# PSilvestre/Clonos

Hardware: AMD Instinct MI355X
Metric: determinants/sec decode+delta-slice (higher is better)
Workload: dtype u8

## Files before the change

### clonos_amd/csrc/decode_fused.hip

```cpp
#include "dev_common.h"
#include "jser_device.h"
#include "jser_flat.h"
#include "handoff.h"

namespace clg {

constexpr uint32_t kZRowDw = kZRegion / 4;
constexpr uint32_t kZPitch = kZRowDw;
constexpr uint32_t kZRows = kZTile / kZRegion + 2;
constexpr uint32_t kZImgDw = kZRows * kZPitch;
constexpr uint32_t kZWin = 1024;
constexpr uint32_t kZEmitWin = 512;
constexpr int kZEmitPair = 1;
constexpr uint32_t kZCanon = 0xFFFFFFFFu;
constexpr uint32_t kZCanonLanes = 16;
constexpr int kZSer = -2;
constexpr uint32_t kZTiny = kZTinySpan;

template <int kCtrl>
__device__ __forceinline__ uint32_t dpp_mov(uint32_t v) {
  return (uint32_t)__builtin_amdgcn_mov_dpp((int)v, kCtrl, 0xF, 0xF, false);
}
__device__ __forceinline__ uint32_t wave_scan_u32(uint32_t v, uint32_t lane) {
  const uint32_t rl = lane & 15u;
// ... 398 lines not shown
template <bool J>
__device__ __forceinline__ Res merge_walk_r(const uint32_t* T, uint32_t re, uint32_t end_a, uint32_t e, const SpecR& s,
                                            const JL& jl) {
  return merge_walk_h(re, end_a, e, s, [&](uint32_t p, uint32_t* Lp, bool* w, uint32_t* why) -> bool {
    const uint32_t tg = zb8(T, p);
    uint32_t L = __builtin_amdgcn_ubfe(kZLutTrue, tg << 2, 4);
    *w = false;
    if (L == 15u || tg >= 8u) {
      int v;
      uint32_t y = 1u;
      if (tg >= 8u) {
        v = (int)kLenErr;
      } else if (tg == CLG_TAG_SERIALIZABLE) {
        if (J) {
          const uint32_t jv = jl_len(jl, p);
          v = jv ? (int)jv : (int)kLenErr;
        } else {
          v = (int)kLenErr;
          y = zbe32(T, p + 1) == 0xACED0005u ? 2u : 1u;
        }
      } else {
        v = tg == CLG_TAG_IGNORE_CHECKPOINT ? 13 : zlen_var(T, p, end_a, tg, 0);
      }
      if (v <= 0) {
        *why = y;
        return false;
      }
      L = (uint32_t)v;
      *w = true;
    }
    *Lp = L;
    return true;
  });
}

__device__ __forceinline__ Res merge_walk_lean(const uint32_t* T, uint32_t re, uint32_t end_a, uint32_t e,
                                               const SpecR& s) {
  Res r{{0, 0}, {0, 0}, e, 0, 0, 0};
  if (e >= re) return r;
  const uint32_t r0 = (re - 1u) & ~(kZRegion - 1u);
  uint32_t p = e, why = 0;
  Bits pb{0, 0}, pw{0, 0};
  auto run = [&](uint64_t sbw, uint64_t& pbw, uint64_t& pww, uint32_t lim) -> uint32_t {
    while (p < lim) {
      constexpr uint32_t kLo = 2u | 9u << 8 | 5u << 16;
      constexpr uint32_t kHi = 5u << 24;
      const uint32_t b = p & 63u;
      const uint64_t m = 1ull << b;
      const bool conv = (sbw & m) != 0ull && p >= s.bad;
      const uint32_t tg = zb8(T, p);
      const uint32_t L = __builtin_amdgcn_perm(kHi, kLo, min(tg, 12u)) & 0xFFu;
      if (conv || L == 0u || p + L > end_a) {
        if (conv) return 1u;
        int v;
        uint32_t y = 1u;
        if (tg >= 8u) {
          v = (int)kLenErr;
        } else if (tg == CLG_TAG_SERIALIZABLE) {
          v = (int)kLenErr;
          y = zbe32(T, p + 1) == 0xACED0005u ? 2u : 1u;
        } else if (L) {
          v = (int)kLenErr;
        } else {
          v = tg == CLG_TAG_IGNORE_CHECKPOINT ? 13 : zlen_var(T, p, end_a, tg, 0);
        }
        if (v <= 0 || p + (uint32_t)v > end_a || p + (uint32_t)v < p) {
          why = v <= 0 ? y : 1u;
          return 2u;
        }
        pbw |= m;
        pww |= m;
        p += (uint32_t)v;
        ++r.steps;
        continue;
      }
      pbw |= m;
      p += L;
      ++r.steps;
    }
    return 0u;
  };
  const uint32_t mid = re < r0 + 64u ? re : r0 + 64u;
  uint32_t st = run(s.sb.lo, pb.lo, pw.lo, mid);
  if (st == 0u) st = run(s.sb.hi, pb.hi, pw.hi, re);
  if (st == 1u) {
    const uint32_t i = p & 127u;
    r.bm = bor(pb, bge(s.sb, i));
    r.wb = bor(pw, bge(s.wb, i));
    r.exit = s.exit;
  } else if (st == 2u) {
    r.bad = why;
    r.exit = s.exit;
    r.bm = pb;
    r.wb = pw;
    r.fail = p;
  } else {
    r.bm = pb;
    r.wb = pw;
    r.exit = p;
  }
  return r;
}

__device__ __forceinline__ uint64_t ld_agent(const uint64_t* p) {
  return __hip_atomic_load(const_cast<uint64_t*>(p), __ATOMIC_RELAXED, __HIP_MEMORY_SCOPE_AGENT);
}
__device__ __forceinline__ uint32_t ld_agent32(const uint32_t* p) {
  return __hip_atomic_load(const_cast<uint32_t*>(p), __ATOMIC_RELAXED, __HIP_MEMORY_SCOPE_AGENT);
}
__device__ __forceinline__ void st_agent(uint64_t* p, uint64_t v) {
  __hip_atomic_store(p, v, __ATOMIC_RELAXED, __HIP_MEMORY_SCOPE_AGENT);
}
__device__ __forceinline__ void note_error(const FusedCtl& ctl, uint32_t span, uint64_t so) {
  if (ctl.span_err && so != ~0ull) atomicMin(reinterpret_cast<unsigned long long*>(ctl.span_err + span), (unsigned long long)so);
}
__device__ __forceinline__ void raise_abort(const FusedCtl& c, ZAbort reason, uint32_t t) {
  __hip_atomic_store(c.abort + kZAbortAny, 1u, __ATOMIC_RELAXED, __HIP_MEMORY_SCOPE_AGENT);
  __hip_atomic_fetch_max(c.abort + reason, ~t, __ATOMIC_RELAXED, __HIP_MEMORY_SCOPE_AGENT);
}

constexpr uint64_t kZSpinLimit = 1ull << 29;
__device__ __forceinline__ bool backoff(uint32_t& n, uint64_t t0) {
  for (uint32_t i = 0; i < n; ++i) __builtin_amdgcn_s_sleep(32);
  n = n < 16u ? n * 2u : 16u;
  return __builtin_amdgcn_s_memtime() - t0 < kZSpinLimit;
}

__device__ __forceinline__ uint64_t pack_cnt(uint32_t rec, uint32_t wide) { return (uint64_t)wide << 31 | rec; }

typedef uint32_t u32x4 __attribute__((ext_vector_type(4)));
constexpr int kZLoads = (int)(kZTile / 16 / 64);
struct StagePre {
  u32x4 v[kZLoads];
  u32x4 hv[2];
  uint32_t hb;
};
template <uint32_t kHaloMax = kZHalo>
struct StageGeom {
  uint32_t t1, halo, img_end;
  uint64_t after;
  bool near, far;
  __device__ __forceinline__ StageGeom(const TileDesc& td, const SpanDesc& sd, uint32_t t, uint32_t hi,
                                       const TileDesc* n1) {
    t1 = sd.first_tile + sd.n_tiles;
    after = td.span_off + td.len;
    const uint64_t rem = sd.len > after ? sd.len - after : 0;
    halo = rem < (uint64_t)kHaloMax ? (uint32_t)rem : kHaloMax;
    img_end = hi + halo;
    const bool next_ok = n1 && halo && t + 1 < t1 && n1->span_off == after && n1->len >= halo;
    near = kHaloMax <= 64u && next_ok;
    far = kHaloMax > 64u && next_ok;
  }
};
template <uint32_t kHaloMax = kZHalo>
__device__ __forceinline__ void stage_issue(const TileDesc& td, const SpanDesc& sd, const uint32_t t, const uint32_t lane,
                                            const uint32_t hi, const TileDesc* n1, StagePre& P) {
  static_assert(kHaloMax <= 64u * 16u * 2u - 32u, "halo words: two per lane");
  const StageGeom<kHaloMax> G(td, sd, t, hi, n1);
  const uint32_t words = (hi + 15) >> 4;
  const CLG_GLOBAL u32x4* src = gp(reinterpret_cast<const u32x4*>(td.abase));
#pragma unroll
  for (int i = 0; i < kZLoads; ++i) {
    const uint32_t w = lane + 64u * (uint32_t)i;
    P.v[i] = src[w < words ? w : words - 1u];
  }
  P.hb = 0;
  if (G.near && lane < G.halo) P.hb = gp(n1->abase)[n1->delta + lane];
  if (G.far) {
    const uint32_t nw = (n1->delta + G.halo + 15u) >> 4;
    const CLG_GLOBAL u32x4* src1 = gp(reinterpret_cast<const u32x4*>(n1->abase));
    P.hv[0] = lane < nw ? src1[lane] : u32x4{0, 0, 0, 0};
    P.hv[1] = lane + 64u < nw ? src1[lane + 64u] : u32x4{0, 0, 0, 0};
  }
}

template <uint32_t kHaloMax = kZHalo, uint32_t kRows = kZRows>
__device__ __forceinline__ void stage_finish(const TileDesc& td, const SpanDesc& sd, const uint32_t t,
                                             const TileDesc* __restrict__ tiles, uint32_t* s_img, const uint32_t lane,
                                             const uint32_t hi, const TileDesc* n1, const StagePre& P) {
  static_assert((kZTile + 15 + kHaloMax + 64 + 127) / 128 <= kRows, "image rows: tile + halo + zero pad");
  const StageGeom<kHaloMax> G(td, sd, t, hi, n1);
  const uint32_t t1 = G.t1, halo = G.halo, img_end = G.img_end;
  const uint64_t after = G.after;
  const bool near = G.near, far = G.far;
  const uint32_t hb = P.hb;
  const u32x4* hv = P.hv;
  {
    const uint32_t words = (hi + 15) >> 4;
#pragma unroll
    for (int i = 0; i < kZLoads; ++i) {
      const uint32_t w = lane + 64u * (uint32_t)i;
      if (w < words) {
        uint32_t* d = s_img + (w >> 3) * kZPitch + 4u * (w & 7u);
        d[0] = P.v[i].x;
        d[1] = P.v[i].y;
        d[2] = P.v[i].z;
        d[3] = P.v[i].w;
      }
    }
  }
  __syncthreads();
  {
    uint8_t* bb = reinterpret_cast<uint8_t*>(s_img);
    if (near) {
      if (lane < halo) bb[rb(hi + lane)] = (uint8_t)hb;
    } else if (far && ((hi - n1->delta) & 15u) == 0u) {
      const uint32_t nw = (n1->delta + halo + 15u) >> 4;
#pragma unroll
      for (uint32_t k = 0; k < 2; ++k) {
        const uint32_t c = lane + 64u * k;
        if (c >= nw) continue;
        const uint32_t at = hi - n1->delta + 16u * c;
        if (16u * c >= n1->delta) {
          uint32_t* d = s_img + rk(at >> 2);
          d[0] = hv[k].x;
          d[1] = hv[k].y;
          d[2] = hv[k].z;
          d[3] = hv[k].w;
        } else {
          const uint32_t w[4] = {hv[k].x, hv[k].y, hv[k].z, hv[k].w};
#pragma unroll
          for (uint32_t b = 0; b < 16; ++b)
            if (16u * c + b >= n1->delta) bb[rb(at + b)] = (uint8_t)(w[b >> 2] >> (8u * (b & 3u)));
        }
      }
    } else if (far) {
#pragma unroll
      for (uint32_t k = 0; k < 2; ++k) {
        const uint32_t c = lane + 64u * k;
        const uint32_t w[4] = {hv[k].x, hv[k].y, hv[k].z, hv[k].w};
#pragma unroll
        for (uint32_t b = 0; b < 16; ++b) {
          const uint32_t x = 16u * c + b;
          if (x >= n1->delta && x < n1->delta + halo) bb[rb(hi + x - n1->delta)] = (uint8_t)(w[b >> 2] >> (8u * (b & 3u)));
        }
      }
    } else {
      const TileDesc nn = halo ? tiles[t + 1] : td;
      if (kHaloMax > 64u && halo > 64u && nn.span_off == after && nn.len >= halo) {
        typedef uint32_t u32x4 __attribute__((ext_vector_type(4)));
        for (uint32_t c = lane; 16u * c < nn.delta + halo; c += 64) {
          const u32x4 v = gp(reinterpret_cast<const u32x4*>(nn.abase))[c];
          const uint32_t w[4] = {v.x, v.y, v.z, v.w};
#pragma unroll
          for (uint32_t b = 0; b < 16; ++b) {
            const uint32_t x = 16u * c + b;
            if (x >= nn.delta && x < nn.delta + halo) bb[rb(hi + x - nn.delta)] = (uint8_t)(w[b >> 2] >> (8u * (b & 3u)));
          }
        }
      } else {
        uint32_t k = t + 1;
        for (uint32_t i = lane; i < halo; i += 64) {
          const uint64_t o = after + i;
          while (k + 1 < t1 && o >= tiles[k].span_off + tiles[k].len) ++k;
          const TileDesc nt = tiles[k];
          bb[rb(hi + i)] = gp(nt.abase)[nt.delta + (uint32_t)(o - nt.span_off)];
        }
      }
    }
    bb[rb(img_end + lane)] = 0;
  }
  __syncthreads();
}


template <uint32_t kHaloMax = kZHalo, uint32_t kRows = kZRows>
__device__ __forceinline__ void stage_image(const TileDesc& td, const SpanDesc& sd, const uint32_t t,
                                            const TileDesc* __restrict__ tiles, uint32_t* s_img, const uint32_t lane,
                                            const uint32_t hi, const TileDesc* n1 = nullptr) {
  StagePre P;
  stage_issue<kHaloMax>(td, sd, t, lane, hi, n1, P);
  stage_finish<kHaloMax, kRows>(td, sd, t, tiles, s_img, lane, hi, n1, P);
}

struct ZTile {
  TileDesc td;
  SpanDesc sd;
  uint32_t lo, hi, end_a, rs, re;
  bool first, last;
};
__device__ __forceinline__ ZTile ztile_of(const TileDesc& td, const SpanDesc& sd, uint32_t t, uint32_t lane) {
  ZTile z;
  z.td = td;
  z.sd = sd;
  z.first = t == z.sd.first_tile;
  z.last = t + 1 == z.sd.first_tile + z.sd.n_tiles;
  z.lo = z.td.delta;
  z.hi = z.td.delta + z.td.len;
  const uint64_t ea = z.sd.len - z.td.span_off + z.td.delta;
  z.end_a = ea > 0xFFFFFF00ull ? 0xFFFFFF00u : (uint32_t)ea;
  const uint32_t r0 = lane * kZRegion;
  z.rs = r0 < z.lo ? z.lo : (r0 > z.hi ? z.hi : r0);
  z.re = r0 + kZRegion > z.hi ? z.hi : r0 + kZRegion;
  return z;
}
__device__ __forceinline__ ZTile ztile(const TileDesc* __restrict__ tiles, const SpanDesc* __restrict__ spans, uint32_t t,
                                       uint32_t lane) {
  const TileDesc td = tiles[t];
  return ztile_of(td, spans[td.span], t, lane);
}

constexpr uint32_t kZLmList = 2 * kZJBitsDw + kZJCap;
__device__ __forceinline__ void build_lm(const ZTile& z, uint32_t* T, uint32_t* list, const uint32_t lane) {
  const bool on = z.rs < z.re;
  const uint32_t r0 = lane * kZRegion;
  uint32_t c[kZRowDw];
  uint64_t cw0 = 0, cw1 = 0;
  constexpr bool kCols = true;
  const int32_t jmax = z.hi > z.lo ? ((int32_t)((z.hi - 1u) >> 7) - (int32_t)(lane >> 5)) >> 1 : -1;
  const uint32_t onm = jmax < 0 ? 0u : (jmax >= 31 ? 0xFFFFFFFFu : (2u << jmax) - 1u);
#pragma unroll
  for (uint32_t j = 0; j < kZRowDw; ++j) {
    const uint32_t x = kCols ? T[64u * j + lane] : T[lane * kZPitch + j];
    const uint32_t h = x & 0xF8F8F8F8u;
    const uint32_t zz = (h - 0x01010101u) & ~h & 0x80808080u;
    const uint32_t vm = __builtin_amdgcn_perm(zz << 8, zz, 0x090B080Au);
    c[j] = __builtin_amdgcn_perm(kLmHi, kLmLo, x) & vm;
    const uint64_t f = (uint64_t)((__builtin_amdgcn_perm(kLmCand, 0u, x) & vm) >> (7u - (j & 7u))) << (32u * ((j >> 3) & 1u));
    if (j < 16u) cw0 |= f; else cw1 |= f;
  }
  if (!kCols && !on) cw0 = cw1 = 0;
  const uint32_t nc = (uint32_t)(__popcll(cw0) + __popcll(cw1));
  const uint32_t incl = wave_scan_u32(nc, lane);
  const uint32_t n = min(lane63(incl), kZLmList);
  uint32_t idx = incl - nc;
#pragma unroll 1
  for (uint32_t hh = 0; hh < 2; ++hh) {
    uint64_t m = hh ? cw1 : cw0;
    while (m) {
      const uint32_t i = (uint32_t)__builtin_ctzll(m);
      m &= m - 1u;
      const uint32_t jj = 16u * hh + 8u * (i >> 5) + (i & 7u), b = (i >> 3) & 3u;
      const uint32_t a = kCols ? 4u * (64u * jj + lane) + b : r0 + 4u * jj + b;
      if (idx < kZLmList) list[idx] = (kCols ? a >= z.lo && a < z.hi : a >= z.rs && a < z.re) ? a : 0xFFFFu;
      ++idx;
    }
  }
  __syncthreads();
  for (uint32_t k = lane; k < n; k += 64) {
    const uint32_t a = list[k];
    const uint32_t code = a != 0xFFFFu ? lm_code(zlen_var(T, a, z.end_a, zb(T, a), 0u), true) : 0u;
    list[k] = a | code << 16;
  }
  __syncthreads();
#pragma unroll
  for (uint32_t j = 0; j < kZRowDw; ++j)
    if ((onm >> j) & 1u) T[64u * j + lane] = c[j];
  __syncthreads();
  for (uint32_t k = lane; k < n; k += 64) {
    const uint32_t e = list[k];
    if (e >> 16) lm8_set(T, e & 0xFFFFu, e >> 16);
  }
  if (on && z.end_a < r0 + kZRegion + 13u) {
    for (uint32_t a = z.end_a > r0 + 13u ? z.end_a - 13u : r0; a < r0 + kZRegion; ++a) {
      const uint32_t cc = lm8(T, a);
      if (a + (cc & 0x7Fu) > z.end_a) lm8_set(T, a, 0u);
    }
  }
}

struct GSpan {
  const TileDesc* tiles;
  uint32_t t, t1, lo;
  uint64_t so;
  __device__ uint32_t at(uint32_t a) const {
    const uint64_t o = so + (a - lo);
    uint32_t k = t;
    while (k + 1 < t1 && o >= tiles[k].span_off + tiles[k].len) ++k;
    const TileDesc d = tiles[k];
    return gp(d.abase)[d.delta + (uint32_t)(o - d.span_off)];
  }
};
struct GRec {
  GSpan g;
  uint32_t base;
  __device__ int operator()(uint64_t k) const { return (int)g.at(base + (uint32_t)k); }
};
__device__ __forceinline__ uint32_t fld_be32(const GRec& b, uint32_t k) {
  return (uint32_t)b(k) << 24 | (uint32_t)b(k + 1) << 16 | (uint32_t)b(k + 2) << 8 | (uint32_t)b(k + 3);
}
__device__ __forceinline__ int lm_true_slow(const GSpan& g, uint32_t p, uint32_t end_a, const JL& jl, uint32_t* wide) {
  const uint32_t tg = g.at(p);
  *wide = is_wide((int)tg);
  if (tg == CLG_TAG_SERIALIZABLE) {
    const uint32_t v = jl_len(jl, p);
    return v ? (int)v : -1;
  }
  const int64_t L = len_fields(GRec{g, p}, (int)tg, (uint64_t)(end_a - p));
  return (L > 0 && L <= 0x7FFFFFF0ll) ? (int)L : -1;
}

__device__ __forceinline__ Res merge_walk_lm(const uint32_t* M, uint32_t re, uint32_t end_a, uint32_t e, const SpecR& s,
                                             const JL& jl, const GSpan& g) {
  return merge_walk_h(re, end_a, e, s, [&](uint32_t p, uint32_t* Lp, bool* w, uint32_t* why) -> bool {
    const uint32_t cc = lm8(M, p);
    uint32_t L = cc & 0x7Fu, wu = cc >> 7;
    if (!L) {
      const int v = lm_true_slow(g, p, end_a, jl, &wu);
      if (v <= 0) {
        *why = 1;
        return false;
      }
      L = (uint32_t)v;
    }
    *Lp = L;
    *w = wu != 0;
    return true;
  });
}

template <bool J>
__device__ __forceinline__ uint32_t canon_walk_r(const uint32_t* T, uint32_t re, uint32_t end_a, uint32_t e,
                                                 const SpecR& s, const JL& jl, const GSpan& g) {
  if (e >= re) return e;
  const uint32_t r0 = (re - 1u) & ~(kZRegion - 1u);
  uint32_t p = e;
  while (p < re) {
    const uint32_t i = p - r0;
    if ((((i < 64u ? s.sb.lo : s.sb.hi) >> (i & 63u)) & 1ull) && p >= s.bad) return s.exit;
    uint32_t L;
    int v = 0;
    if (J && jl.lm) {
      const uint32_t c = lm8(jl.lm, p);
      L = c & 0x7Fu;
      if (c == 0x80u) {
        uint32_t w;
        v = lm_true_slow(g, p, end_a, jl, &w);
      }
    } else {
      bool w;
      L = spec_len_fast<J>(T, p, end_a, false, jl, &w);
      if (!L) {
        const uint32_t tg = zb8(T, p);
        if (tg == CLG_TAG_TIMER_TRIGGER || tg == CLG_TAG_SOURCE_CHECKPOINT) v = zlen_var(T, p, end_a, tg, 0u);
        else if (J && tg == CLG_TAG_SERIALIZABLE) v = (int)min(jl_len(jl, p), 0x7FFFFFFFu);
      }
    }
    if (!L) L = (v > 0 && v <= (int)kZTile) ? (uint32_t)v : 1u;
    p += L;
  }
  return p;
}

template <bool J>
__device__ __forceinline__ uint32_t canon_exit_r(const ZTile& z, const uint32_t* s_img, const SpecR& sp, uint32_t lane,
                                                 const JL& jl, const TileDesc* __restrict__ tiles, uint32_t t) {
  const GSpan g{tiles, t, z.sd.first_tile + z.sd.n_tiles, z.lo, z.td.span_off};
  const uint32_t last_l = z.hi > z.lo ? (z.hi - 1) >> 7 : 0;
  const uint32_t c0 = last_l >= kZCanonLanes - 1 ? last_l - (kZCanonLanes - 1) : 0;
  const bool on = lane >= c0 && z.rs < z.re;
  uint32_t cx = on ? sp.exit : z.rs, entry = kZCanon;
  for (int it = 0; it <= 64; ++it) {
    const uint32_t prev = wave_prev_u32(cx);
    const uint32_t want = lane <= c0 ? kZCanon : prev;
    const bool ch = want != entry;
    if (!__any(ch)) break;
    if (ch) {
      entry = want;
      cx = on ? canon_walk_r<J>(s_img, z.re, z.end_a, want, sp, jl, g) : want;
    }
  }
  return lane63(cx);
}

constexpr uint32_t kZWarmFlat = 1u << 31;
__device__ __forceinline__ uint32_t warm_start(uint32_t rs, uint32_t lo, uint32_t warm, uint32_t lane) {
  const uint32_t st = (lane >> 1) & 15u;
  const uint32_t w = (warm & kZWarmFlat) ? (warm & ~kZWarmFlat) : warm + 4u * st;
  return rs >= lo + w ? rs - w : lo;
}

template <bool J>
__device__ __forceinline__ ZAbort count_tile(const uint32_t t, const ZTile& z, const uint32_t e_true,
                                           const uint32_t must_exit, const FusedCtl& ctl, const uint32_t* s_img,
                                           const uint32_t lane, uint32_t* x_out, const JL& jl,
                                           const TileDesc* __restrict__ tiles = nullptr,
                                           const SpecR* walked = nullptr, uint64_t* cnt_out = nullptr,
                                           uint64_t* bm_out = nullptr, uint32_t* fail_out = nullptr) {
#define ZPHASE(i) \
  if (ctl.prof && lane == 0) ctl.prof[(uint64_t)t * 8 + (i)] = __builtin_amdgcn_s_memtime()
  ZPHASE(1);
  const uint32_t lo = z.lo, rs = z.rs, re = z.re, end_a = z.end_a;
  const uint32_t ws = warm_start(rs, lo, ctl.warm, lane), wsb = warm_start(lane * kZRegion + 64u, lo, ctl.warm, lane);
  const SpecR sp = walked ? *walked
                          : rs < re ? spec_walk_fast<J>(s_img, ws, wsb, rs, re, end_a, lane * kZRegion, jl, ctl.lean != 0u)
                                    : SpecR{{0, 0}, {0, 0}, rs, rs, 0};

  ZPHASE(2);
  const uint32_t guess = wave_prev_u32(sp.exit);
  uint32_t entry = lane == 0 ? e_true : guess;
  const GSpan g{tiles, t, z.sd.first_tile + z.sd.n_tiles, lo, z.td.span_off};
  auto merge = [&](uint32_t from) -> Res {
    if (rs >= re) return Res{{0, 0}, {0, 0}, from, 0, 0, 0};
    if (J && jl.lm) return merge_walk_lm(s_img, re, end_a, from, sp, jl, g);
    if (!J && ctl.lean) return merge_walk_lean(s_img, re, end_a, from, sp);
    return merge_walk_r<J>(s_img, re, end_a, from, sp, jl);
  };
  Res r = merge(entry);
  uint32_t steps0 = r.steps, steps_more = 0, iters = 0;
  uint32_t shift = 0;
  for (int it = 0; it <= 64; ++it) {
    const uint32_t prev = wave_prev_u32(r.exit);
    uint32_t want = lane == 0 ? e_true : prev;
    bool ch = want != entry;
    const uint64_t cm = __ballot(ch);
    if (!cm) break;
    ++iters;
    const uint32_t low = (uint32_t)__builtin_ctzll(cm);
    const uint32_t d = (uint32_t)__builtin_amdgcn_readlane((int)(want - entry), (int)low);
    if ((cm & (cm - 1)) == 0 && d == shift && lane > low) {
      want = entry + d;
      ch = true;
    }
    shift = (cm & (cm - 1)) == 0 ? d : 0u;
    if (ch) {
      entry = want;
      r = merge(want);
      steps_more += r.steps;
    }
  }
  if (ctl.prof) {
    uint32_t m0 = steps0, m1 = steps_more;
#pragma unroll
    for (int off = 32; off > 0; off >>= 1) {
      m0 = max(m0, (uint32_t)__shfl_xor(m0, off));
      m1 = max(m1, (uint32_t)__shfl_xor(m1, off));
    }
    if (lane == 0) ctl.prof[(uint64_t)t * 8 + 5] = (uint64_t)m0 | (uint64_t)m1 << 20 | (uint64_t)iters << 40;
  }
  const uint32_t x_true = lane63(r.exit);
  *x_out = x_true;
  const uint64_t badm = __ballot(r.bad != 0u);
  ZAbort reason = badm ? (__shfl(r.bad, (int)__builtin_ctzll(badm)) == 2u ? kZAbortSerializable : kZAbortBad) : kZAbortNone;
  if (z.last) {
    if (x_true != end_a) reason = reason ? reason : kZAbortEnd;
  } else if (must_exit != kZCanon && x_true != must_exit) {
    reason = reason ? reason : kZAbortExit;
  }
  if (reason && ctl.dbg) {
    uint32_t claim = 0;
    if (lane == 0) claim = atomicCAS(ctl.dbg + kZDbgClaim, 0u, 1u) == 0u ? 1u : 0u;
    if (__shfl(claim, 0)) {
      if (lane == 0) {
        ctl.dbg[kZDbgTile] = t; ctl.dbg[kZDbgReason] = reason; ctl.dbg[kZDbgMustExit] = must_exit;
        ctl.dbg[kZDbgXTrue] = x_true; ctl.dbg[kZDbgETrue] = e_true;
        ctl.dbg[kZDbgLo] = lo; ctl.dbg[kZDbgHi] = z.hi; ctl.dbg[kZDbgEndA] = end_a;
      }
      uint32_t* d = ctl.dbg + kZDbgLanes + kZDbgLaneWords * lane;
      d[0] = rs; d[1] = re; d[2] = sp.exit; d[3] = sp.bad; d[4] = sp.first; d[5] = 0; d[6] = entry;
      d[7] = r.exit | r.bad << 31;
    }
  }
  uint32_t fail_a = 0xFFFFFFFFu;
  if (reason == kZAbortBad && badm && ctl.span_err) {
    const uint32_t bl = (uint32_t)__builtin_ctzll(badm);
    fail_a = (uint32_t)__shfl((int)r.fail, (int)bl);
    if (lane > bl) {
      r.bm = Bits{0, 0};
      r.wb = Bits{0, 0};
    }
  }
  if (fail_out) *fail_out = fail_a;
  if (reason && reason != kZAbortExit && fail_a == 0xFFFFFFFFu) return reason;

  ZPHASE(3);
  const uint32_t pk = wave_sum_u32(bcount(r.bm) | bcount(r.wb) << 16);
  const uint32_t rec = pk & 0xFFFFu, wide = pk >> 16;
  if (lane == 0) gp(ctl.cnt)[t] = pack_cnt(rec, wide);
  if (cnt_out) *cnt_out = pack_cnt(rec, wide);
  if (bm_out) {
    bm_out[0] = r.bm.lo;
    bm_out[1] = r.bm.hi;
  }
  if (!bm_out) {
    typedef uint64_t u64x2 __attribute__((ext_vector_type(2)));
    u64x2 out_bits;
    out_bits.x = r.bm.lo;
    out_bits.y = r.bm.hi;
    gp(reinterpret_cast<u64x2*>(ctl.bits))[(uint64_t)t * 64 + lane] = out_bits;
  }
  ZPHASE(4);
#undef ZPHASE
  return reason;
}

__device__ __forceinline__ uint64_t wave_incl_scan(uint64_t v, uint32_t lane) {
#pragma unroll
  for (int off = 1; off < 64; off <<= 1) {
    const uint64_t y = __shfl_up(v, off);
    if ((int)lane >= off) v += y;
  }
  return v;
}

__global__ __launch_bounds__(256) void k_decode_scan1(FusedCtl ctl) {
  __shared__ uint64_t s_w[4];
  if (ld_agent32(ctl.abort + kZAbortAny)) return;
  const uint32_t tid = threadIdx.x, lane = tid & 63u, wv = tid >> 6;
  const uint32_t nt = ctl.n_tiles, blk = blockIdx.x, i0 = blk * kZScanBlock + tid * 4u;
  uint64_t v[4], sum = 0;
#pragma unroll
  for (int j = 0; j < 4; ++j) {
    v[j] = i0 + j < nt ? gp(ctl.cnt)[i0 + j] : 0ull;
    sum += v[j];
  }
  const uint64_t incl = wave_incl_scan(sum, lane);
  if (lane == 63u) s_w[wv] = incl;
  __syncthreads();
  uint64_t run = incl - sum;
  for (uint32_t k = 0; k < wv; ++k) run += s_w[k];
#pragma unroll
  for (int j = 0; j < 4; ++j) {
    if (i0 + j < nt) gp(ctl.base)[i0 + j] = run;
    run += v[j];
  }
  if (tid == 255u) gp(ctl.boff)[blk] = run;
}

__global__ __launch_bounds__(256) void k_decode_scan2(FusedCtl ctl, uint32_t n_blocks) {
  __shared__ uint64_t s_w[4];
  if (ld_agent32(ctl.abort + kZAbortAny)) return;
  const uint32_t tid = threadIdx.x, lane = tid & 63u, wv = tid >> 6, i0 = 4u * tid;
  uint64_t v[4], sum = 0;
#pragma unroll
  for (int j = 0; j < 4; ++j) {
    v[j] = i0 + j < n_blocks ? gp(ctl.boff)[i0 + j] : 0ull;
    sum += v[j];
  }
  const uint64_t incl = wave_incl_scan(sum, lane);
  if (lane == 63u) s_w[wv] = incl;
  __syncthreads();
  uint64_t run = incl - sum;
  for (uint32_t k = 0; k < wv; ++k) run += s_w[k];
#pragma unroll
  for (int j = 0; j < 4; ++j) {
    if (i0 + j < n_blocks) gp(ctl.boff)[i0 + j] = run;
    run += v[j];
// ... 361 lines not shown
        for (uint32_t j = 0; j < 9; ++j) d[j] = s_img[rk(k0 + j)];
#pragma unroll
        for (uint32_t j = 0; j < 8; ++j) x[j] = __builtin_amdgcn_alignbit(d[j + 1], d[j], sh);
        auto be32 = [&](uint32_t off) {
          return __builtin_bswap32(__builtin_amdgcn_alignbyte(x[(off >> 2) + 1], x[off >> 2], off & 3u));
        };
        const uint32_t tg = x[0] & 0xFFu;
        const bool ser = tg == CLG_TAG_SERIALIZABLE, tt = tg == CLG_TAG_TIMER_TRIGGER, sc = tg == CLG_TAG_SOURCE_CHECKPOINT;
        const uint32_t b13 = (x[3] >> 8) & 0xFFu, b21 = (x[5] >> 8) & 0xFFu, b22 = (x[5] >> 16) & 0xFFu;
        const bool tt_name = tt && b13 == 6u, sc_ref = sc && b22 != 0u;
        const uint32_t jlen = J && ser ? jl_len_bits(jl, a) : 0u;
        const uint32_t L = ser ? jlen : tt_name ? 18u + be32(14) : tt ? 14u : sc_ref ? 27u + be32(23) : sc ? 23u : 13u;
        const uint32_t var_off = ser ? 1u : tt_name ? 18u : sc_ref ? 27u : 0u;
        const int64_t v0 = ser ? (int64_t)L - 1 : (int64_t)((uint64_t)be32(5) << 32 | be32(9));
        if (fits || g < out.cap) o_v0[w0 + i] = v0;
        const uint64_t wi = wide + k;
        if (wi < out.wcap) {
          const uint32_t so = (uint32_t)(td.span_off + (a - lo));
          gp(out.w_idx)[wi] = (uint32_t)g;
          gp(out.w_rc)[wi] = ser ? 0 : (int32_t)be32(1);
          gp(out.w_v1)[wi] = sc ? (int64_t)((uint64_t)be32(13) << 32 | be32(17)) : 0;
          gp(out.w_var_off)[wi] = var_off ? so + var_off : 0u;
          gp(out.w_var_len)[wi] = var_off ? L - var_off : 0u;
          gp(out.w_sub)[wi] = (uint8_t)(tt ? b13 : sc ? (b21 | (sc_ref ? 0x80u : 0u)) : 0u);
        }
      }
    }
    wide += nwide;
    __syncthreads();
  }
}

template <bool J>
__global__ __launch_bounds__(64) void k_decode_emit(const TileDesc* __restrict__ tiles, const SpanDesc* __restrict__ spans,
                                                    FusedCtl ctl, DecodeOut out) {
  __shared__ EmitLds<J> L;
  const uint32_t t = blockIdx.x, lane = threadIdx.x;
  if (ld_agent32(ctl.abort + kZAbortAny)) return;
  if (ctl.lb_check && t && t % kZScanBlock == 0 && lane == 0) lookback_check(ctl, t / kZScanBlock);
  if (ctl.skip_bad && gp(ctl.span_bad)[tiles[t].span]) return;
  if (ctl.span_err && tiles[t].span_off > gp(ctl.span_err)[tiles[t].span]) return;
  emit_tile<J>(tiles, spans, ctl, out, t, lane, gp(ctl.base)[t] + gp(ctl.boff)[t / kZScanBlock], L);
}

constexpr uint64_t kZTinyDone = 1ull << 62;
__device__ __forceinline__ bool tiny_tile(const TileDesc& td, const SpanDesc& sd) {
  return sd.n_tiles == 1 && td.span_off == 0 && td.len > 0 && td.len <= kZTiny && td.len == sd.len;
}
__global__ __launch_bounds__(64) void k_decode_count_tiny(const TileDesc* __restrict__ tiles,
                                                          const SpanDesc* __restrict__ spans, FusedCtl ctl) {
  const uint32_t ti = blockIdx.x * 64 + threadIdx.x;
  if (ti >= ctl.n_tiles) return;
  const TileDesc td = tiles[ti];
  if (!tiny_tile(td, spans[td.span]) || (ctl.skip_bad && gp(ctl.span_bad)[td.span])) return;
  constexpr uint32_t kLeave = 3u;
  uint32_t why = 0, rec = 0, wide = 0;
  typedef uint32_t u32x4 __attribute__((ext_vector_type(4)));
  typedef uint64_t u64x2 __attribute__((ext_vector_type(2)));
  const CLG_GLOBAL u32x4* src = gp(reinterpret_cast<const u32x4*>(td.abase));
  auto* bits = gp(reinterpret_cast<u64x2*>(ctl.bits)) + (uint64_t)ti * 64;
  const uint32_t end = td.delta + td.len;
  uint32_t a = td.delta, wb = 0xFFFFFFFFu, cur = 0;
  u32x4 w{};
  uint64_t blo = 0, bhi = 0;
  constexpr uint32_t kLut = 2u | 9u << 4 | 5u << 8 | 13u << 24 | 5u << 28;
  while (a < end) {
    if ((a >> 4) != wb) {
      wb = a >> 4;
      w = src[wb];
    }
    const uint32_t q = a & 15u;
    const uint32_t dw = q < 8u ? (q < 4u ? w.x : w.y) : (q < 12u ? w.z : w.w);
    const uint32_t tg = (dw >> (8u * (q & 3u))) & 0xFFu;
    const uint32_t L = tg < 8u ? (kLut >> (4u * tg)) & 0xFu : 0u;
    if (!L) {
      why = (tg == CLG_TAG_SERIALIZABLE || tg == CLG_TAG_TIMER_TRIGGER || tg == CLG_TAG_SOURCE_CHECKPOINT) ? kLeave : kZAbortBad;
      break;
    }
    if (a + L > end) {
      why = kZAbortBad;
      break;
    }
    for (const uint32_t r = a >> 7; cur < r; ++cur) {
      u64x2 v;
      v.x = blo;
      v.y = bhi;
      bits[cur] = v;
      blo = bhi = 0;
    }
    const uint32_t i = a & 127u;
    if (i < 64u) blo |= 1ull << i; else bhi |= 1ull << (i - 64u);
    ++rec;
    wide += tg == CLG_TAG_IGNORE_CHECKPOINT ? 1u : 0u;
    a += L;
  }
  if (why == kLeave) return;
  if (why == 0u || ctl.span_err) {
    for (const uint32_t r = (end - 1) >> 7; cur <= r; ++cur) {
      u64x2 v;
      v.x = blo;
      v.y = bhi;
      bits[cur] = v;
      blo = bhi = 0;
    }
    gp(ctl.cnt)[ti] = pack_cnt(rec, wide);
  }
  if (why) {
    raise_abort(ctl, ZAbort(why), ti);
    if (ctl.span_bad) __hip_atomic_store(ctl.span_bad + td.span, 1u, __ATOMIC_RELAXED, __HIP_MEMORY_SCOPE_AGENT);
    note_error(ctl, td.span, (uint64_t)(a - td.delta));
  }
  gp(ctl.st_x)[ti] = kZTinyDone;
}

constexpr uint64_t kZExValid = 1ull << 63;
constexpr uint64_t kZExFail = 1ull << 62;

__device__ __forceinline__ void push_repair(const FusedCtl& ctl, uint32_t c) {
  gp(ctl.rep_flag)[c] = 1u;
  atomicAdd(ctl.rep + kZRepFiled, 1u);
}
__device__ __forceinline__ void mark_bad(const FusedCtl& ctl, ZAbort reason, uint32_t t, uint32_t span) {
  raise_abort(ctl, reason, t);
  if (ctl.span_bad) __hip_atomic_store(ctl.span_bad + span, 1u, __ATOMIC_RELAXED, __HIP_MEMORY_SCOPE_AGENT);
}
__device__ __forceinline__ uint32_t chunk_first(const FusedCtl& ctl, uint32_t c, uint32_t K, uint32_t G) {
  if (c >= G) return ctl.n_tiles;
  return ctl.chunk ? ctl.chunk[c] : min(ctl.n_tiles, c * K);
}
__device__ __forceinline__ void check_chunk(const FusedCtl& ctl, const TileDesc* __restrict__ tiles, uint32_t f,
                                            uint32_t ce, uint32_t lane) {
  const uint32_t span = tiles[f].span;
  uint32_t bad = 0xFFFFFFFFu;
  for (uint32_t i = f + lane; i < ce; i += 64) {
    if (tiles[i].span != span) break;
    if (!(ld_agent(&ctl.ex[i]) & kZExValid)) {
      bad = i;
      break;
    }
  }
  const uint64_t m = __ballot(bad != 0xFFFFFFFFu);
  if (m && lane == (uint32_t)__builtin_ctzll(m)) {
    mark_bad(ctl, kZAbortBad, bad, span);
    const uint64_t e = ld_agent(&ctl.ex[bad]);
    if (e & kZExFail) note_error(ctl, span, e & ~kZExFail);
  }
}

template <bool J>
__device__ __forceinline__ ZAbort count_staged(const TileDesc* __restrict__ tiles, const SpanDesc* __restrict__ spans,
                                                 const FusedCtl& ctl, uint32_t* s_img, uint32_t* s_j, uint32_t lane,
                                                 uint32_t t, const ZTile& z, uint64_t xs, uint32_t must_exit,
                                                 const SpecR* walked, uint64_t* x, uint64_t* cnt_out = nullptr,
                                                 uint64_t* bm_out = nullptr, uint64_t* fail_so = nullptr) {
  const uint32_t nt = ctl.n_tiles;
  const TileDesc n1 = tiles[t + 1 < nt ? t + 1 : t];
  const uint64_t ee = xs - z.td.span_off + z.lo;
  const uint32_t e_true = ee > 0xFFFFFF00ull ? 0xFFFFFF00u : (uint32_t)ee;
  JL jl{nullptr, nullptr, nullptr};
  JLPre pre{};
  if (J) pre = jl_prefetch(ctl, t, lane);
  stage_image(z.td, z.sd, t, tiles, s_img, lane, z.hi, &n1);
  if (J) build_lm(z, s_img, s_j, lane);
  if (J) jl = load_jl_map(ctl, t, s_j, lane, s_img, pre);
  uint32_t x_true, fa = 0xFFFFFFFFu;
  const ZAbort why = count_tile<J>(t, z, e_true, must_exit, ctl, s_img, lane, &x_true, jl, tiles, walked, cnt_out,
                                   bm_out, fail_so ? &fa : nullptr);
  *x = z.td.span_off + (x_true - z.lo);
  if (fail_so) *fail_so = fa != 0xFFFFFFFFu ? z.td.span_off + (fa - z.lo) : ~0ull;
  return why;
}

constexpr uint32_t kZWalkDisagree = 4;

__device__ __forceinline__ bool zero_tile_walk(const ZTile& z, uint64_t xs, const FusedCtl& ctl, uint32_t t,
                                               uint32_t lane, uint64_t* x) {
  const uint32_t words = (z.hi + 15) >> 4;
  const CLG_GLOBAL u32x4* src = gp(reinterpret_cast<const u32x4*>(z.td.abase));
  uint32_t any = 0;
#pragma unroll
  for (int i = 0; i < kZLoads; ++i) {
    const uint32_t w = lane + 64u * (uint32_t)i;
    const u32x4 v = src[w < words ? w : words - 1u];
    any |= v.x | v.y | v.z | v.w;
  }
  if (__any(any != 0u)) return false;
  const uint32_t e = (uint32_t)(xs - z.td.span_off) + z.lo;
  const uint32_t n = (z.hi - e + 1u) >> 1;
  const uint32_t r0 = lane * kZRegion;
  const uint64_t pat = (e & 1u) ? 0xAAAAAAAAAAAAAAAAull : 0x5555555555555555ull;
  auto word = [&](uint32_t b0) -> uint64_t {
    uint64_t m = pat;
    if (e > b0) m = e - b0 >= 64u ? 0ull : m & (~0ull << (e - b0));
    if (z.hi < b0 + 64u) m = z.hi <= b0 ? 0ull : m & ((1ull << (z.hi - b0)) - 1ull);
    return m;
  };
  typedef uint64_t u64x2 __attribute__((ext_vector_type(2)));
  u64x2 bits;
  bits.x = word(r0);
  bits.y = word(r0 + 64u);
  gp(reinterpret_cast<u64x2*>(ctl.bits))[(uint64_t)t * 64 + lane] = bits;
  if (lane == 0) gp(ctl.cnt)[t] = pack_cnt(n, 0);
  *x = z.td.span_off + (e + 2u * n - z.lo);
  return true;
}

__device__ __forceinline__ bool wrong_entry(const FusedCtl& ctl, uint32_t c, uint32_t f) {
  const uint64_t e = ld_agent(&ctl.ent[c]);
  if (!pk_state(e) || f == 0) return false;
  const uint64_t xe = ld_agent(&ctl.ex[f - 1]);
  return !(xe & kZExValid) || (xe & ~kZExValid) != pk_val(e);
}

template <bool J>
__device__ __forceinline__ bool serve_chunk(const TileDesc* __restrict__ tiles, const SpanDesc* __restrict__ spans,
                                            const FusedCtl& ctl, uint32_t* s_img, uint32_t* s_j, uint32_t lane,
                                            uint32_t c, uint32_t f, uint32_t ce, uint32_t* walk_end) {
  if (f == 0 || f >= ce || tiles[f].span_off == 0) return true;
  if (f >= *walk_end) {
    const uint64_t xe = ld_agent(&ctl.ex[f - 1]);
    if (!(xe & kZExValid)) {
      if (lane == 0) mark_bad(ctl, kZAbortBad, f - 1, tiles[f].span);
      return true;
    }
    uint64_t xs = xe & ~kZExValid;
    const uint64_t e = ld_agent(&ctl.ent[c]);
    const uint64_t taken = pk_state(e) ? pk_val(e) : pk_val(ld_agent(&ctl.st_x[f - 1]));
    if (xs != taken) {
      uint32_t disagree = 0;
      for (uint32_t t = f; t < ctl.n_tiles; ++t) {
        const ZTile z = ztile(tiles, spans, t, lane);
        *walk_end = t + 1;
        uint64_t x = xs, fso = ~0ull;
        ZAbort why = kZAbortNone;
        bool zero = false;
        if (!z.last && xs >= z.td.span_off + z.td.len) {
          typedef uint64_t u64x2 __attribute__((ext_vector_type(2)));
          gp(reinterpret_cast<u64x2*>(ctl.bits))[(uint64_t)t * 64 + lane] = u64x2{0, 0};
          if (lane == 0) gp(ctl.cnt)[t] = 0;
        } else if (!z.last && zero_tile_walk(z, xs, ctl, t, lane, &x)) {
          zero = true;
        } else {
          why = count_staged<J>(tiles, spans, ctl, s_img, s_j, lane, t, z, xs, kZCanon, nullptr, &x, nullptr, nullptr,
                                &fso);
          __syncthreads();
          if (why == kZAbortBad && lane == 0) note_error(ctl, z.td.span, fso);
        }
        if (why) {
          if (lane == 0) {
            mark_bad(ctl, why, t, z.td.span);
            st_agent(&ctl.ex[t], why == kZAbortBad && fso != ~0ull ? kZExFail | fso : 0ull);
          }
          break;
        }
        const uint64_t xv = kZExValid | x;
        uint32_t old = 0;
        if (lane == 0) {
          const uint64_t o = ld_agent(&ctl.ex[t]);
          old = o == xv ? 1u : (o & kZExValid) ? 2u : 0u;
          st_agent(&ctl.ex[t], xv);
          if (ctl.dbg) {
            uint64_t* w = reinterpret_cast<uint64_t*>(ctl.dbg + kZDbgTiles) + 2 * (uint64_t)t;
            w[0] = xs;
            w[1] = 2ull << 60 | (uint64_t)blockIdx.x << 32 | (uint64_t)(f & 0xFFFFFF) << 4 | old;
          }
        }
        old = __shfl(old, 0);
        if (old == 1u || z.last) break;
        if (old == 2u && !zero && ++disagree > kZWalkDisagree) {
          if (lane == 0) {
            mark_bad(ctl, kZAbortExit, t, z.td.span);
            if (ctl.dbg) {
              ctl.dbg[kZDbgWalkMark] = kZDbgWalkGaveUp; ctl.dbg[kZDbgWalkFrom] = f; ctl.dbg[kZDbgWalkAt] = t;
              ctl.dbg[kZDbgWalkEntry] = (uint32_t)(xs - z.td.span_off);
              ctl.dbg[kZDbgWalkExit] = (uint32_t)(x - z.td.span_off); ctl.dbg[kZDbgWalkSpan] = z.td.span;
              ctl.dbg[kZDbgWalkDisagree] = disagree;
            }
          }
          return false;
        }
        xs = x;
      }
    }
  }
  check_chunk(ctl, tiles, f, ce, lane);
  return true;
}

template <bool J>
constexpr int kZCountWaves = J ? 3 : 4;
template <bool J>
__global__ __launch_bounds__(64) __attribute__((amdgpu_waves_per_eu(kZCountWaves<J>))) void k_decode_count(const TileDesc* __restrict__ tiles, const SpanDesc* __restrict__ spans,
                                                     FusedCtl ctl) {
  __shared__ uint32_t s_img[kZImgDw];
  __shared__ uint32_t s_j[J ? 2 * kZJBitsDw + kZJCap : 1];
  const uint32_t lane = threadIdx.x, nt = ctl.n_tiles;
  JL jl{nullptr, nullptr, nullptr};
  const uint32_t K = (nt + gridDim.x - 1) / gridDim.x;
  const uint32_t t0 = chunk_first(ctl, blockIdx.x, K, gridDim.x), t1 = chunk_first(ctl, blockIdx.x + 1, K, gridDim.x);
  uint32_t x_pub = kZCanon;
  SpecR sp_last{{0, 0}, {0, 0}, 0, 0, 0};
  if (t0 < t1) {
    const ZTile z = ztile(tiles, spans, t1 - 1, lane);
    if (!z.last && t1 < nt) {
      stage_image(z.td, z.sd, t1 - 1, tiles, s_img, lane, z.hi);
      if (J) build_lm(z, s_img, s_j, lane);
      if (J) jl = load_jl_map(ctl, t1 - 1, s_j, lane, s_img, jl_prefetch(ctl, t1 - 1, lane));
      const uint32_t ws = warm_start(z.rs, z.lo, ctl.warm, lane);
      const uint32_t wsb = warm_start(lane * kZRegion + 64u, z.lo, ctl.warm, lane);
      sp_last = z.rs < z.re ? spec_walk_fast<J>(s_img, ws, wsb, z.rs, z.re, z.end_a, lane * kZRegion, jl, ctl.lean != 0u)
                            : SpecR{{0, 0}, {0, 0}, z.rs, z.rs, 0};
      x_pub = canon_exit_r<J>(z, s_img, sp_last, lane, jl, tiles, t1 - 1);
      if (x_pub < z.hi) {
        if (lane == 0) atomicAdd(ctl.rep + kZRepCanonEarly, 1u);
        x_pub = z.hi;
      }
      if (lane == 0) st_agent(&ctl.st_x[t1 - 1], pk_word(2u, (uint64_t)z.td.span_off + (x_pub - z.lo)));
      __syncthreads();
    }
  }
  uint64_t x_prev = 0;
  uint32_t bad_span = 0xFFFFFFFFu;
  uint32_t sus_span = 0xFFFFFFFFu;
  for (uint32_t t = t0; t < t1; ++t) {
    const ZTile z = ztile(tiles, spans, t, lane);
    if (z.td.span == bad_span) continue;
    if (!J && ctl.tiny && z.first && z.last && z.td.len <= kZTiny && gp(ctl.st_x)[t] == kZTinyDone)
      continue;
    if (ctl.prof && lane == 0) ctl.prof[(uint64_t)t * 8] = __builtin_amdgcn_s_memtime();
    uint64_t xs;
    if (z.first) {
      xs = z.td.span_off;
    } else if (t > t0) {
      xs = x_prev;
    } else {
      uint64_t v;
      uint32_t nb = 1;
      const uint64_t w0 = __builtin_amdgcn_s_memtime();
      for (;;) {
        v = ld_agent(&ctl.st_x[t - 1]);
        if (pk_state(v) && pk_val(v) >= z.td.span_off) break;
        if (pk_state(v) && ctl.dbg && lane == 0) {
          if (atomicAdd(ctl.dbg + kZDbgSkipN, 1u) == 0u) {
            ctl.dbg[kZDbgSkipTile] = t; ctl.dbg[kZDbgSkipWordLo] = (uint32_t)v; ctl.dbg[kZDbgSkipWordHi] = (uint32_t)(v >> 32);
            ctl.dbg[kZDbgSkipOff] = (uint32_t)z.td.span_off; ctl.dbg[kZDbgSkipPolls] = nb;
          }
        }
        if (ld_agent32(ctl.abort + kZAbortTimeout)) return;
        if (!backoff(nb, w0)) {
          if (lane == 0) raise_abort(ctl, kZAbortTimeout, t);
          return;
        }
      }
      xs = pk_val(v) + (ctl.perturb & 0xFFFFu);
      sus_span = z.td.span;
      if (lane == 0) st_agent(&ctl.ent[blockIdx.x], pk_word(2u, xs));
    }
    const bool reuse = t + 1 == t1 && x_pub != kZCanon;
    uint64_t x;
    uint64_t fso = ~0ull;
    const ZAbort why = count_staged<J>(tiles, spans, ctl, s_img, s_j, lane, t, z, xs, t + 1 == t1 ? x_pub : kZCanon,
                                       reuse ? &sp_last : nullptr, &x, nullptr, nullptr, &fso);
    if (why == kZAbortNone || why == kZAbortExit) {
      x_prev = x;
      if (lane == 0) {
        st_agent(&ctl.ex[t], kZExValid | x);
        if (ctl.dbg) {
          uint64_t* w = reinterpret_cast<uint64_t*>(ctl.dbg + kZDbgTiles) + 2 * (uint64_t)t;
          w[0] = xs;
          w[1] = 1ull << 60 | (uint64_t)blockIdx.x << 32 | (uint64_t)(t0 & 0xFFFFFF) << 4 | why;
        }
        if (why == kZAbortExit) {
          uint32_t c = blockIdx.x + 1;
          while (chunk_first(ctl, c + 1, K, gridDim.x) == t1) ++c;
          push_repair(ctl, c);
        }
      }
    } else {
      const bool soft = why != kZAbortSerializable && z.td.span == sus_span;
      if (lane == 0) {
        if (soft) {
          push_repair(ctl, blockIdx.x);
          if (why == kZAbortBad && fso != ~0ull) st_agent(&ctl.ex[t], kZExFail | fso);
        } else {
          mark_bad(ctl, why, t, z.td.span);
          if (why == kZAbortBad) note_error(ctl, z.td.span, fso);
        }
      }
      if (!soft && !ctl.span_bad) return;
      if (soft)
        x_prev = z.td.span_off + z.td.len;
      else
        bad_span = z.td.span;
    }
    __syncthreads();
  }
}

template <bool J>
__global__ __launch_bounds__(64) void k_decode_repair(const TileDesc* __restrict__ tiles, const SpanDesc* __restrict__ spans,
                                                      FusedCtl ctl) {
  __shared__ uint32_t s_img[kZImgDw];
  __shared__ uint32_t s_j[J ? 2 * kZJBitsDw + kZJCap : 1];
  if (ld_agent32(ctl.abort + kZAbortTimeout) || ld_agent32(ctl.abort + kZAbortSerializable) ||
      ld_agent32(ctl.abort + kZAbortOverflow))
    return;
  const uint32_t G = gridDim.x, b = blockIdx.x, lane = threadIdx.x, K = (ctl.n_tiles + G - 1) / G;
  const uint32_t fb = chunk_first(ctl, b, K, G);
  if (fb >= chunk_first(ctl, b + 1, K, G)) return;
  auto need = [&](uint32_t c, uint32_t f) -> bool { return gp(ctl.rep_flag)[c] || wrong_entry(ctl, c, f); };
  if (!need(b, fb)) return;
  const uint32_t span = tiles[fb].span;
  for (uint32_t hi = b; hi > 0;) {
    const uint32_t lo = hi > 64u ? hi - 64u : 0u, k = lo + lane;
    const bool in = k < hi;
    const uint32_t ft = in ? chunk_first(ctl, k, K, G) : 0u;
    const uint32_t kt = in ? chunk_first(ctl, k + 1, K, G) : 0u;
    const bool empty = in && kt == ft, same = in && !empty && tiles[ft].span == span;
    if (__any(same && need(k, ft))) return;
    if (!__all(!in || empty || same)) break;
    hi = lo;
  }
  uint32_t walk_end = 0;
  for (uint32_t c = b; c < G; ++c) {
    const uint32_t f = chunk_first(ctl, c, K, G), ce = chunk_first(ctl, c + 1, K, G);
    if (f >= ce) continue;
    if (tiles[f].span != span) break;
    if (!gp(ctl.rep_flag)[c]) {
      if (!wrong_entry(ctl, c, f)) continue;
      if (lane == 0 && (ld_agent(&ctl.ex[f - 1]) & kZExValid)) atomicAdd(ctl.rep + kZRepServed, 1u);
    }
    if (!serve_chunk<J>(tiles, spans, ctl, s_img, s_j, lane, c, f, ce, &walk_end)) break;
  }
}

constexpr uint32_t kZAggSet = 2u, kZAggBad = 3u;

__device__ __forceinline__ void decode_small_tiles(const TileDesc* __restrict__ tiles,
                                                   const SpanDesc* __restrict__ spans, uint32_t nt, const FusedCtl& ctl,
                                                   const DecodeOut& out, uint64_t* agg, uint64_t* agg_next,
                                                   uint64_t* res) {
  __shared__ EmitLds<false, true> L;
  const uint32_t t = blockIdx.x, lane = threadIdx.x;
  for (uint32_t j = t + nt * lane; j < kZSmallAggWords; j += 64u * nt) agg_next[j] = 0;
  const ZTile z = ztile(tiles, spans, t, lane);
  const TileDesc n1 = tiles[t + 1 < nt ? t + 1 : t];
  stage_image(z.td, z.sd, t, tiles, L.img, lane, z.hi, &n1);
  const JL jl{nullptr, nullptr, nullptr};
  const uint32_t ws = warm_start(z.rs, z.lo, ctl.warm, lane), wsb = warm_start(lane * kZRegion + 64u, z.lo, ctl.warm, lane);
  const SpecR sp = z.rs < z.re ? spec_walk_fast<false>(L.img, ws, wsb, z.rs, z.re, z.end_a, lane * kZRegion, jl,
                                                       ctl.lean != 0u)
                               : SpecR{{0, 0}, {0, 0}, z.rs, z.rs, 0};
  uint64_t xs = z.td.span_off;
  bool bad = false;
  if (!z.first) {
    uint64_t v = 0;
    if (lane == 0) {
      const uint64_t w0 = __builtin_amdgcn_s_memtime();
      while (!pk_state(v = ld_agent(&agg[nt + t - 1]))) {
        __builtin_amdgcn_s_sleep(1);
        if (__builtin_amdgcn_s_memtime() - w0 >= kZSpinLimit) {
          v = pk_word(kZAggBad, 0);
          break;
        }
      }
    }
    v = ((uint64_t)__builtin_amdgcn_readfirstlane((uint32_t)(v >> 32)) << 32) |
        (uint32_t)__builtin_amdgcn_readfirstlane((uint32_t)v);
    bad = pk_state(v) == kZAggBad;
    xs = pk_val(v) + (ctl.perturb & 0xFFFFu);
  }
  uint64_t c = 0, x = 0, bm[2] = {0, 0};
  if (!bad) {
    const uint64_t ee = xs - z.td.span_off + z.lo;
    const uint32_t e_true = ee > 0xFFFFFF00ull ? 0xFFFFFF00u : (uint32_t)ee;
    uint32_t x_true;
    const ZAbort why = count_tile<false>(t, z, e_true, kZCanon, ctl, L.img, lane, &x_true, jl, tiles, &sp, &c, bm);
    x = z.td.span_off + (x_true - z.lo);
    bad = why != kZAbortNone;
  }
  if (lane == 0) {
    st_agent(&agg[nt + t], pk_word(bad ? kZAggBad : kZAggSet, x));
    st_agent(&agg[t], pk_word(bad ? kZAggBad : kZAggSet, c));
  }
  uint64_t pre = 0;
  bool any_bad = bad;
  for (uint32_t j0 = 0; j0 < t && !any_bad; j0 += 64) {
    const uint32_t j = j0 + lane;
    uint64_t v = 0;
    if (j < t) {
      const uint64_t w0 = __builtin_amdgcn_s_memtime();
      while (!pk_state(v = ld_agent(&agg[j]))) {
        __builtin_amdgcn_s_sleep(1);
        if (__builtin_amdgcn_s_memtime() - w0 >= kZSpinLimit) {
          v = pk_word(kZAggBad, 0);
          break;
        }
      }
    }
    any_bad = __any(pk_state(v) == kZAggBad);
    uint64_t cj = pk_val(v);
#pragma unroll
    for (int off = 32; off > 0; off >>= 1) cj += __shfl_xor(cj, off);
    pre += cj;
  }
  if (any_bad) {
    if (lane == 0) __hip_atomic_store(res + kZSmallFailed, 1ull, __ATOMIC_RELAXED, __HIP_MEMORY_SCOPE_SYSTEM);
    return;
  }
  emit_tile<false, true>(tiles, spans, ctl, out, t, lane, pre, L, bm);
  if (lane == 0) {
    uint64_t* ck = res + small_check_at(ctl.n_spans, t);
    ck[kZCheckEntryExit] = (uint64_t)(uint32_t)xs | (uint64_t)(uint32_t)x << 32;
    ck[kZCheckBase] = pre;
    ck[kZCheckCount] = c;
// ... 539 lines not shown
```

Baseline: 98.38 billion.

## Stage only the canonical tail of the last tile and raise count-kernel occupancy

Result: no change. 99.55 billion, median of 5 (+1.2%).

```diff
diff --git a/clonos_amd/csrc/decode_fused.hip b/clonos_amd/csrc/decode_fused.hip
--- a/clonos_amd/csrc/decode_fused.hip
+++ b/clonos_amd/csrc/decode_fused.hip
@@ -574,16 +574,17 @@
     far = kHaloMax > 64u && next_ok;
   }
 };
-template <uint32_t kHaloMax = kZHalo>
+template <uint32_t kHaloMax = kZHalo, int kLoads = kZLoads>
 __device__ __forceinline__ void stage_issue(const TileDesc& td, const SpanDesc& sd, const uint32_t t, const uint32_t lane,
-                                            const uint32_t hi, const TileDesc* n1, StagePre& P) {
+                                            const uint32_t hi, const TileDesc* n1, StagePre& P, const uint32_t w0 = 0) {
+  static_assert(kLoads <= kZLoads, "the words a lane holds");
   static_assert(kHaloMax <= 64u * 16u * 2u - 32u, "halo words: two per lane");
   const StageGeom<kHaloMax> G(td, sd, t, hi, n1);
   const uint32_t words = (hi + 15) >> 4;
   const CLG_GLOBAL u32x4* src = gp(reinterpret_cast<const u32x4*>(td.abase));
 #pragma unroll
-  for (int i = 0; i < kZLoads; ++i) {
-    const uint32_t w = lane + 64u * (uint32_t)i;
+  for (int i = 0; i < kLoads; ++i) {
+    const uint32_t w = w0 + lane + 64u * (uint32_t)i;
     P.v[i] = src[w < words ? w : words - 1u];
   }
   P.hb = 0;
@@ -596,10 +597,11 @@
   }
 }
 
-template <uint32_t kHaloMax = kZHalo, uint32_t kRows = kZRows>
+template <uint32_t kHaloMax = kZHalo, uint32_t kRows = kZRows, int kLoads = kZLoads>
 __device__ __forceinline__ void stage_finish(const TileDesc& td, const SpanDesc& sd, const uint32_t t,
                                              const TileDesc* __restrict__ tiles, uint32_t* s_img, const uint32_t lane,
-                                             const uint32_t hi, const TileDesc* n1, const StagePre& P) {
+                                             const uint32_t hi, const TileDesc* n1, const StagePre& P,
+                                             const uint32_t w0 = 0) {
   static_assert((kZTile + 15 + kHaloMax + 64 + 127) / 128 <= kRows, "image rows: tile + halo + zero pad");
   const StageGeom<kHaloMax> G(td, sd, t, hi, n1);
   const uint32_t t1 = G.t1, halo = G.halo, img_end = G.img_end;
@@ -610,8 +612,8 @@
   {
     const uint32_t words = (hi + 15) >> 4;
 #pragma unroll
-    for (int i = 0; i < kZLoads; ++i) {
-      const uint32_t w = lane + 64u * (uint32_t)i;
+    for (int i = 0; i < kLoads; ++i) {
+      const uint32_t w = w0 + lane + 64u * (uint32_t)i;
       if (w < words) {
         uint32_t* d = s_img + (w >> 3) * kZPitch + 4u * (w & 7u);
         d[0] = P.v[i].x;
@@ -686,13 +688,13 @@
 }
 
 
-template <uint32_t kHaloMax = kZHalo, uint32_t kRows = kZRows>
+template <uint32_t kHaloMax = kZHalo, uint32_t kRows = kZRows, int kLoads = kZLoads>
 __device__ __forceinline__ void stage_image(const TileDesc& td, const SpanDesc& sd, const uint32_t t,
                                             const TileDesc* __restrict__ tiles, uint32_t* s_img, const uint32_t lane,
-                                            const uint32_t hi, const TileDesc* n1 = nullptr) {
+                                            const uint32_t hi, const TileDesc* n1 = nullptr, const uint32_t w0 = 0) {
   StagePre P;
-  stage_issue<kHaloMax>(td, sd, t, lane, hi, n1, P);
-  stage_finish<kHaloMax, kRows>(td, sd, t, tiles, s_img, lane, hi, n1, P);
+  stage_issue<kHaloMax, kLoads>(td, sd, t, lane, hi, n1, P, w0);
+  stage_finish<kHaloMax, kRows, kLoads>(td, sd, t, tiles, s_img, lane, hi, n1, P, w0);
 }
 
 struct ZTile {
@@ -864,12 +866,16 @@
   return p;
 }
 
+__device__ __forceinline__ uint32_t canon_first_lane(const ZTile& z) {
+  const uint32_t last_l = z.hi > z.lo ? (z.hi - 1) >> 7 : 0;
+  return last_l >= kZCanonLanes - 1 ? last_l - (kZCanonLanes - 1) : 0;
+}
+
 template <bool J>
 __device__ __forceinline__ uint32_t canon_exit_r(const ZTile& z, const uint32_t* s_img, const SpecR& sp, uint32_t lane,
                                                  const JL& jl, const TileDesc* __restrict__ tiles, uint32_t t) {
   const GSpan g{tiles, t, z.sd.first_tile + z.sd.n_tiles, z.lo, z.td.span_off};
-  const uint32_t last_l = z.hi > z.lo ? (z.hi - 1) >> 7 : 0;
-  const uint32_t c0 = last_l >= kZCanonLanes - 1 ? last_l - (kZCanonLanes - 1) : 0;
+  const uint32_t c0 = canon_first_lane(z);
   const bool on = lane >= c0 && z.rs < z.re;
   uint32_t cx = on ? sp.exit : z.rs, entry = kZCanon;
   for (int it = 0; it <= 64; ++it) {
@@ -898,13 +904,14 @@
                                            const uint32_t lane, uint32_t* x_out, const JL& jl,
                                            const TileDesc* __restrict__ tiles = nullptr,
                                            const SpecR* walked = nullptr, uint64_t* cnt_out = nullptr,
-                                           uint64_t* bm_out = nullptr, uint32_t* fail_out = nullptr) {
+                                           uint64_t* bm_out = nullptr, uint32_t* fail_out = nullptr,
+                                           const uint32_t walked_from = 0) {
 #define ZPHASE(i) \
   if (ctl.prof && lane == 0) ctl.prof[(uint64_t)t * 8 + (i)] = __builtin_amdgcn_s_memtime()
   ZPHASE(1);
   const uint32_t lo = z.lo, rs = z.rs, re = z.re, end_a = z.end_a;
   const uint32_t ws = warm_start(rs, lo, ctl.warm, lane), wsb = warm_start(lane * kZRegion + 64u, lo, ctl.warm, lane);
-  const SpecR sp = walked ? *walked
+  const SpecR sp = walked && lane >= walked_from ? *walked
                           : rs < re ? spec_walk_fast<J>(s_img, ws, wsb, rs, re, end_a, lane * kZRegion, jl, ctl.lean != 0u)
                                     : SpecR{{0, 0}, {0, 0}, rs, rs, 0};
 
@@ -1572,7 +1579,8 @@
                                                  const FusedCtl& ctl, uint32_t* s_img, uint32_t* s_j, uint32_t lane,
                                                  uint32_t t, const ZTile& z, uint64_t xs, uint32_t must_exit,
                                                  const SpecR* walked, uint64_t* x, uint64_t* cnt_out = nullptr,
-                                                 uint64_t* bm_out = nullptr, uint64_t* fail_so = nullptr) {
+                                                 uint64_t* bm_out = nullptr, uint64_t* fail_so = nullptr,
+                                                 const uint32_t walked_from = 0) {
   const uint32_t nt = ctl.n_tiles;
   const TileDesc n1 = tiles[t + 1 < nt ? t + 1 : t];
   const uint64_t ee = xs - z.td.span_off + z.lo;
@@ -1585,7 +1593,7 @@
   if (J) jl = load_jl_map(ctl, t, s_j, lane, s_img, pre);
   uint32_t x_true, fa = 0xFFFFFFFFu;
   const ZAbort why = count_tile<J>(t, z, e_true, must_exit, ctl, s_img, lane, &x_true, jl, tiles, walked, cnt_out,
-                                   bm_out, fail_so ? &fa : nullptr);
+                                   bm_out, fail_so ? &fa : nullptr, walked_from);
   *x = z.td.span_off + (x_true - z.lo);
   if (fail_so) *fail_so = fa != 0xFFFFFFFFu ? z.td.span_off + (fa - z.lo) : ~0ull;
   return why;
@@ -1708,7 +1716,8 @@
 }
 
 template <bool J>
-constexpr int kZCountWaves = J ? 3 : 4;
+constexpr int kZCountWaves = J ? 3 : 5;
+constexpr int kZTailLoads = 3;
 template <bool J>
 __global__ __launch_bounds__(64) __attribute__((amdgpu_waves_per_eu(kZCountWaves<J>))) void k_decode_count(const TileDesc* __restrict__ tiles, const SpanDesc* __restrict__ spans,
                                                      FusedCtl ctl) {
@@ -1718,18 +1727,27 @@
   JL jl{nullptr, nullptr, nullptr};
   const uint32_t K = (nt + gridDim.x - 1) / gridDim.x;
   const uint32_t t0 = chunk_first(ctl, blockIdx.x, K, gridDim.x), t1 = chunk_first(ctl, blockIdx.x + 1, K, gridDim.x);
-  uint32_t x_pub = kZCanon;
+  uint32_t x_pub = kZCanon, sp_from = 0;
   SpecR sp_last{{0, 0}, {0, 0}, 0, 0, 0};
   if (t0 < t1) {
     const ZTile z = ztile(tiles, spans, t1 - 1, lane);
     if (!z.last && t1 < nt) {
-      stage_image(z.td, z.sd, t1 - 1, tiles, s_img, lane, z.hi);
+      const uint32_t c0 = canon_first_lane(z);
+      const uint32_t rs0 = max(c0 * kZRegion, z.lo);
+      const uint32_t w0 = warm_start(rs0, z.lo, ctl.warm, c0) >> 4, words = (z.hi + 15) >> 4;
+      if (!J && words - w0 <= 64u * (uint32_t)kZTailLoads) {
+        stage_image<kZHalo, kZRows, kZTailLoads>(z.td, z.sd, t1 - 1, tiles, s_img, lane, z.hi, nullptr, w0);
+        sp_from = c0;
+      } else {
+        stage_image(z.td, z.sd, t1 - 1, tiles, s_img, lane, z.hi);
+      }
       if (J) build_lm(z, s_img, s_j, lane);
       if (J) jl = load_jl_map(ctl, t1 - 1, s_j, lane, s_img, jl_prefetch(ctl, t1 - 1, lane));
       const uint32_t ws = warm_start(z.rs, z.lo, ctl.warm, lane);
       const uint32_t wsb = warm_start(lane * kZRegion + 64u, z.lo, ctl.warm, lane);
-      sp_last = z.rs < z.re ? spec_walk_fast<J>(s_img, ws, wsb, z.rs, z.re, z.end_a, lane * kZRegion, jl, ctl.lean != 0u)
-                            : SpecR{{0, 0}, {0, 0}, z.rs, z.rs, 0};
+      sp_last = z.rs < z.re && lane >= sp_from
+                    ? spec_walk_fast<J>(s_img, ws, wsb, z.rs, z.re, z.end_a, lane * kZRegion, jl, ctl.lean != 0u)
+                    : SpecR{{0, 0}, {0, 0}, z.rs, z.rs, 0};
       x_pub = canon_exit_r<J>(z, s_img, sp_last, lane, jl, tiles, t1 - 1);
       if (x_pub < z.hi) {
         if (lane == 0) atomicAdd(ctl.rep + kZRepCanonEarly, 1u);
@@ -1777,10 +1795,11 @@
       if (lane == 0) st_agent(&ctl.ent[blockIdx.x], pk_word(2u, xs));
     }
     const bool reuse = t + 1 == t1 && x_pub != kZCanon;
+    const SpecR* const walked = J ? (reuse ? &sp_last : nullptr) : &sp_last;
     uint64_t x;
     uint64_t fso = ~0ull;
     const ZAbort why = count_staged<J>(tiles, spans, ctl, s_img, s_j, lane, t, z, xs, t + 1 == t1 ? x_pub : kZCanon,
-                                       reuse ? &sp_last : nullptr, &x, nullptr, nullptr, &fso);
+                                       walked, &x, nullptr, nullptr, &fso, reuse ? sp_from : 64u);
     if (why == kZAbortNone || why == kZAbortExit) {
       x_prev = x;
       if (lane == 0) {
```
